# pqpeqr/RL-2048-with-Reinforce-and-Actor-Critic

Hardware: AMD Instinct MI355X
Metric: env steps/sec (whole node) + achieved HBM GB/s, batch=1M 4x4 boards (higher is better)
Workload: dtype u64

## Files before the change

rl-2048-with-reinforce-and-actor-critic_amd/csrc/g2048_dw2.hip:

```cpp
#include <hip/hip_runtime.h>

#include "g2048.h"

namespace {

typedef float floatx16 __attribute__((ext_vector_type(16)));
typedef __bf16 bf16x8 __attribute__((ext_vector_type(8)));

constexpr int kBK = 16;
constexpr int kAhead = 2;
constexpr int kStages = kAhead + 2;
constexpr int kThreads = 256;

__host__ __device__ inline int acc_row(int r, int h) { return (r & 3) + 8 * (r >> 2) + 4 * h; }

__device__ __forceinline__ void glds16(const float* src, float* lds_wave_base) {
#if defined(__HIP_DEVICE_COMPILE__)
    const uint32_t lds = __builtin_amdgcn_readfirstlane(
        (uint32_t)(uintptr_t)(__attribute__((address_space(3))) float*)lds_wave_base);
    uint32_t keep;
    asm volatile("s_mov_b32 %0, m0\n\ts_mov_b32 m0, %2\n\ts_nop 0\n\tglobal_load_lds_dwordx4 %1, off\n\ts_mov_b32 m0, %0"
                 : "=&s"(keep)
                 : "v"(src), "s"(lds)
                 : "memory");
#else
    (void)src;
    (void)lds_wave_base;
#endif
}

__host__ __device__ constexpr int dw2_threads(int nt2) { return nt2 >= 8 ? 512 : 256; }

template <int NT1, int NT2, int MODE>
struct Dw2 {
    static constexpr bool FAC = MODE != 0;
    static constexpr int H1 = 32 * NT1, H2 = 32 * NT2;
    static constexpr int RB = H1 > H2 ? H1 : H2;
    static constexpr bool WIDE = NT2 >= 8;
    static constexpr int CS = 1;
    static constexpr int kW = WIDE ? 8 : 4;
    static constexpr int WR = 2, WC = kW / 2;
    static constexpr int kThr = 64 * kW;
    static_assert(kThr == dw2_threads(NT2), "launch bounds");
    static constexpr int NT2h = NT2 / CS, H2h = H2 / CS;
    static constexpr int kRows = FAC ? H1 : H1 + H2h;
    static constexpr int kRecFloats = FAC ? 256 : 0;
    static constexpr int kStageFloats = kRows * kBK + kRecFloats;
    static constexpr int kRowGlds = kRows / 16;
    static constexpr int kGlds = kRowGlds + (FAC ? 1 : 0);
    static constexpr int kGldsPerWave = (kGlds + kW - 1) / kW;
    static constexpr int TR = NT1 >= WR ? NT1 / WR : 1;
    static constexpr int TC = NT2h >= WC ? NT2h / WC : 1;
};

struct Dw2Args {
    const float* a1t;
    const float* d2t;
    const float* w3;
    float* part;
    uint32_t ld, col0, ncols, kb;
};


__device__ __forceinline__ void split3(const float (&v)[8], bf16x8& p0, bf16x8& p1, bf16x8& p2) {
#pragma unroll
    for (int j = 0; j < 8; j++) {
        const __bf16 h = (__bf16)v[j];
        const float r = v[j] - (float)h;
        const __bf16 m = (__bf16)r;
        const float r2 = r - (float)m;
        p0[j] = h;
        p1[j] = m;
        p2[j] = (__bf16)r2;
    }
}

__device__ __forceinline__ void read_frag(const float* stage, int row, int h, float (&v)[8]) {
    const int f = (row >> 2) & 3;
    const float4 x = *reinterpret_cast<const float4*>(stage + row * kBK + (((2 * h) ^ f) << 2));
    const float4 y = *reinterpret_cast<const float4*>(stage + row * kBK + (((2 * h + 1) ^ f) << 2));
    v[0] = x.x; v[1] = x.y; v[2] = x.z; v[3] = x.w;
    v[4] = y.x; v[5] = y.y; v[6] = y.z; v[7] = y.w;
}

template <int NT1, int NT2, int MODE>
__global__ void __launch_bounds__(dw2_threads(NT2), 1) dw2_kernel(Dw2Args a) {
    using G = Dw2<NT1, NT2, MODE>;
    constexpr bool FAC = G::FAC;
    __shared__ float S[kStages * G::kStageFloats];
    const int t = threadIdx.x, lane = t & 63, w = t >> 6, h = lane >> 5, r = lane & 31;
    const int wr = w / G::WC, wc = w % G::WC;
    const uint32_t k_begin = a.col0 + blockIdx.x * a.kb;
    const uint32_t k_end = min(k_begin + a.kb, a.col0 + a.ncols);
    const int iters = k_end > k_begin ? (int)((k_end - k_begin) / kBK) : 0;
    const int c0 = (int)blockIdx.y * G::H2h;

    const int ws = __builtin_amdgcn_readfirstlane(w);
    const auto glds_index = [&](int i) {
        const int g = ws + G::kW * i;
        return g < G::kGlds ? g : G::kGlds - 1;
    };
    const float* src[G::kGldsPerWave];
#pragma unroll
    for (int i = 0; i < G::kGldsPerWave; i++) {
        const int g = glds_index(i);
        if (FAC && g == G::kRowGlds) {
            src[i] = a.d2t + (size_t)(k_begin / kBK) * 256 + 4 * lane;
        } else {
            const int row = 16 * g + (lane >> 2);
            const int chunk = (lane & 3) ^ ((lane >> 4) & 3);
            const float* base = row < G::H1 ? a.a1t + row * kBK : a.d2t + (row - G::H1 + c0) * kBK;
            src[i] = base + (size_t)(k_begin / kBK) * G::RB * kBK + 4 * chunk;
        }
    }
    const auto issue_to = [&](int slot, int stage_idx) {
        float* dst = S + slot * G::kStageFloats;
#pragma unroll
        for (int i = 0; i < G::kGldsPerWave; i++) {
            const int g = glds_index(i);
            const uint32_t stride = (FAC && g == G::kRowGlds) ? 256u : (uint32_t)(G::RB * kBK);
            glds16(src[i] + (size_t)stage_idx * stride, dst + 16 * g * kBK);
        }
    };

    floatx16 acc[G::TR][G::TC];
#pragma unroll
    for (int i = 0; i < G::TR; i++)
#pragma unroll
        for (int j = 0; j < G::TC; j++) acc[i][j] = floatx16{};
    const bool rows_mine = NT1 >= G::WR || wr == 0, cols_mine = G::NT2h >= G::WC || wc == 0;
    const int drow = G::H1 + (t < G::H2h ? t : G::H2h - 1);
    const int dunit = c0 + (t < G::H2h ? t : G::H2h - 1);
    float dsum = 0.0f;
    float4 w3d = make_float4(0.f, 0.f, 0.f, 0.f), w3c[G::TC];
    if constexpr (MODE == 2) {
        const float4* w3v = reinterpret_cast<const float4*>(a.w3);
        w3d = w3v[dunit];
#pragma unroll
        for (int j = 0; j < G::TC; j++) w3c[j] = w3v[c0 + 32 * ((G::NT2h >= G::WC ? wc : 0) * G::TC + j) + r];
    }
    const auto d2_of = [](const float4 g, const float4 w, bool m) {
        float dh = g.x * w.x;
        dh = fmaf(g.y, w.y, dh);
        dh = fmaf(g.z, w.z, dh);
        dh = fmaf(g.w, w.w, dh);
        return dh * (m ? 1.0f : 0.0f);
    };

    struct Planes {
        bf16x8 a0[G::TR], a1[G::TR], a2[G::TR], b0[G::TC], b1[G::TC], b2[G::TC];
    };
    typedef unsigned int u32x4 __attribute__((ext_vector_type(4)));
    const auto load = [&](const float* st, Planes& p) {
        if constexpr (MODE == 2) {
            const float* rec = st + G::kRows * kBK;
            const uint16_t* mw = reinterpret_cast<const uint16_t*>(rec);
            const float4* gv = reinterpret_cast<const float4*>(rec + 128);
            {
                const uint32_t m = mw[dunit];
#pragma unroll
                for (int e = 0; e < 16; e++) dsum += d2_of(gv[e], w3d, (m >> e) & 1u);
            }
            if (rows_mine && cols_mine) {
#pragma unroll
                for (int i = 0; i < G::TR; i++) {
                    float v[8];
                    read_frag(st, 32 * (wr * G::TR + i) + r, h, v);
                    split3(v, p.a0[i], p.a1[i], p.a2[i]);
                }
                float4 gk[8];
#pragma unroll
                for (int e = 0; e < 8; e++) gk[e] = gv[8 * h + e];
#pragma unroll
                for (int j = 0; j < G::TC; j++) {
                    const uint32_t m = (uint32_t)mw[c0 + 32 * (wc * G::TC + j) + r] >> (8 * h);
                    float v[8];
#pragma unroll
                    for (int e = 0; e < 8; e++) v[e] = d2_of(gk[e], w3c[j], (m >> e) & 1u);
                    split3(v, p.b0[j], p.b1[j], p.b2[j]);
                }
            }
            return;
        }
        if constexpr (MODE == 1) {
            const float* rec = st + G::kRows * kBK;
            const uint16_t* mw = reinterpret_cast<const uint16_t*>(rec);
            const float* gv = rec + 128;
            {
                const uint32_t m = mw[dunit];
#pragma unroll
                for (int c = 0; c < 4; c++) {
                    const float4 x = *reinterpret_cast<const float4*>(gv + 4 * c);
                    dsum += ((m >> (4 * c + 0)) & 1u) ? x.x : 0.0f;
                    dsum += ((m >> (4 * c + 1)) & 1u) ? x.y : 0.0f;
                    dsum += ((m >> (4 * c + 2)) & 1u) ? x.z : 0.0f;
                    dsum += ((m >> (4 * c + 3)) & 1u) ? x.w : 0.0f;
                }
            }
            if (rows_mine && cols_mine) {
                const float4 g0 = *reinterpret_cast<const float4*>(gv + 8 * h);
                const float4 g1 = *reinterpret_cast<const float4*>(gv + 8 * h + 4);
                const float gk[8] = {g0.x, g0.y, g0.z, g0.w, g1.x, g1.y, g1.z, g1.w};
#pragma unroll
                for (int i = 0; i < G::TR; i++) {
                    float v[8];
                    read_frag(st, 32 * (wr * G::TR + i) + r, h, v);
#pragma unroll
                    for (int e = 0; e < 8; e++) v[e] *= gk[e];
                    split3(v, p.a0[i], p.a1[i], p.a2[i]);
                }
#pragma unroll
                for (int j = 0; j < G::TC; j++) {
                    const uint32_t m = (uint32_t)mw[c0 + 32 * (wc * G::TC + j) + r] >> (8 * h);
                    u32x4 q;
#pragma unroll
                    for (int e = 0; e < 4; e++)
                        q[e] = (((m >> (2 * e)) & 1u) * 0x3F80u) | (((m >> (2 * e + 1)) & 1u) * 0x3F800000u);
                    p.b0[j] = __builtin_bit_cast(bf16x8, q);
                }
            }
            return;
        }
        const float* rowp = st + drow * kBK;
#pragma unroll
        for (int c = 0; c < 4; c++) {
            const float4 x = *reinterpret_cast<const float4*>(rowp + 4 * c);
            dsum += x.x;
            dsum += x.y;
            dsum += x.z;
            dsum += x.w;
        }
        if (rows_mine && cols_mine) {
#pragma unroll
            for (int i = 0; i < G::TR; i++) {
                float v[8];
                read_frag(st, 32 * (wr * G::TR + i) + r, h, v);
                split3(v, p.a0[i], p.a1[i], p.a2[i]);
            }
#pragma unroll
            for (int j = 0; j < G::TC; j++) {
                float v[8];
                read_frag(st, G::H1 + 32 * (wc * G::TC + j) + r, h, v);
                split3(v, p.b0[j], p.b1[j], p.b2[j]);
            }
        }
    };
    const auto mfma = [&](const Planes& p) {
        if (rows_mine && cols_mine) {
#pragma unroll
            for (int i = 0; i < G::TR; i++)
#pragma unroll
                for (int j = 0; j < G::TC; j++) {
                    floatx16 c = acc[i][j];
                    if constexpr (MODE == 1) {
                        c = __builtin_amdgcn_mfma_f32_32x32x16_bf16(p.a2[i], p.b0[j], c, 0, 0, 0);
                        c = __builtin_amdgcn_mfma_f32_32x32x16_bf16(p.a1[i], p.b0[j], c, 0, 0, 0);
                        c = __builtin_amdgcn_mfma_f32_32x32x16_bf16(p.a0[i], p.b0[j], c, 0, 0, 0);
                        acc[i][j] = c;
                        continue;
                    }
                    c = __builtin_amdgcn_mfma_f32_32x32x16_bf16(p.a2[i], p.b0[j], c, 0, 0, 0);
                    c = __builtin_amdgcn_mfma_f32_32x32x16_bf16(p.a1[i], p.b1[j], c, 0, 0, 0);
                    c = __builtin_amdgcn_mfma_f32_32x32x16_bf16(p.a0[i], p.b2[j], c, 0, 0, 0);
                    c = __builtin_amdgcn_mfma_f32_32x32x16_bf16(p.a1[i], p.b0[j], c, 0, 0, 0);
                    c = __builtin_amdgcn_mfma_f32_32x32x16_bf16(p.a0[i], p.b1[j], c, 0, 0, 0);
                    c = __builtin_amdgcn_mfma_f32_32x32x16_bf16(p.a0[i], p.b0[j], c, 0, 0, 0);
                    acc[i][j] = c;
                }
        }
    };
    const auto step = [&](int it, const Planes& cur, Planes& nxt) {
        const int q = it + 1 + kAhead;
        issue_to(q % kStages, q < iters ? q : iters - 1);
        asm volatile("s_waitcnt vmcnt(%0)" ::"n"(kAhead * G::kGldsPerWave) : "memory");
        __builtin_amdgcn_s_barrier();
        asm volatile("" ::: "memory");
        load(S + ((it + 1) % kStages) * G::kStageFloats, nxt);
        mfma(cur);
        constexpr int kMfma = (MODE == 1 ? 3 : 6) * G::TR * G::TC;
        __builtin_amdgcn_sched_group_barrier(0x100, 8, 0);
#pragma unroll
        for (int m = 0; m < kMfma; m++) {
            __builtin_amdgcn_sched_group_barrier(0x008, 1, 0);
            __builtin_amdgcn_sched_group_barrier(0x100, 1, 0);
            __builtin_amdgcn_sched_group_barrier(0x002, 4, 0);
        }
    };

    if constexpr (G::WIDE) {
        Planes pa;
        if (iters > 0) {
#pragma unroll
            for (int q = 0; q < kAhead; q++) issue_to(q, q < iters ? q : iters - 1);
            for (int it = 0; it < iters; it++) {
                const int q = it + kAhead;
                issue_to(q % kStages, q < iters ? q : iters - 1);
                asm volatile("s_waitcnt vmcnt(%0)" ::"n"(kAhead * G::kGldsPerWave) : "memory");
                __builtin_amdgcn_s_barrier();
                asm volatile("" ::: "memory");
                load(S + (it % kStages) * G::kStageFloats, pa);
                mfma(pa);
            }
            asm volatile("s_waitcnt vmcnt(0)" ::: "memory");
        }
    } else {
    Planes pa, pb;
    if (iters > 0) {
#pragma unroll
        for (int q = 0; q <= kAhead; q++) issue_to(q, q < iters ? q : iters - 1);
        asm volatile("s_waitcnt vmcnt(%0)" ::"n"(kAhead * G::kGldsPerWave) : "memory");
        __builtin_amdgcn_s_barrier();
        asm volatile("" ::: "memory");
        load(S, pa);
        int it = 0;
        for (; it + 2 < iters; it += 2) {
            step(it, pa, pb);
            step(it + 1, pb, pa);
        }
        if (it + 1 < iters) {
            step(it, pa, pb);
            mfma(pb);
        } else {
            mfma(pa);
        }
        asm volatile("s_waitcnt vmcnt(0)" ::: "memory");
    }
    }
    float* out = a.part + (size_t)blockIdx.x * (G::H1 + 1) * G::H2;
    if (rows_mine && cols_mine) {
#pragma unroll
        for (int j = 0; j < G::TC; j++) {
            const float ws = MODE == 1 ? a.w3[c0 + 32 * (wc * G::TC + j) + r] : 1.0f;
#pragma unroll
            for (int i = 0; i < G::TR; i++)
#pragma unroll
                for (int q = 0; q < 16; q++)
                    out[(size_t)(32 * (wr * G::TR + i) + acc_row(q, h)) * G::H2 + c0 + 32 * (wc * G::TC + j) + r] =
                        MODE == 1 ? acc[i][j][q] * ws : acc[i][j][q];
        }
    }
    if (t < G::H2h) out[(size_t)G::H1 * G::H2 + dunit] = MODE == 1 ? dsum * a.w3[dunit] : dsum;
}

template <int NT1, int MODE>
void launch_nt2(const Dw2Args& a, int nt2, int grid, hipStream_t s) {
    switch (nt2) {
        case 1: hipLaunchKernelGGL((dw2_kernel<NT1, 1, MODE>), dim3(grid, Dw2<NT1, 1, MODE>::CS), dim3(Dw2<NT1, 1, MODE>::kThr), 0, s, a); break;
        case 2: hipLaunchKernelGGL((dw2_kernel<NT1, 2, MODE>), dim3(grid, Dw2<NT1, 2, MODE>::CS), dim3(Dw2<NT1, 2, MODE>::kThr), 0, s, a); break;
        case 4: hipLaunchKernelGGL((dw2_kernel<NT1, 4, MODE>), dim3(grid, Dw2<NT1, 4, MODE>::CS), dim3(Dw2<NT1, 4, MODE>::kThr), 0, s, a); break;
        default: hipLaunchKernelGGL((dw2_kernel<NT1, 8, MODE>), dim3(grid, Dw2<NT1, 8, MODE>::CS), dim3(Dw2<NT1, 8, MODE>::kThr), 0, s, a); break;
    }
}

template <int NT1>
void launch_mode(const Dw2Args& a, int mode, int nt2, int grid, hipStream_t s) {
    if (mode == 1) launch_nt2<NT1, 1>(a, nt2, grid, s);
    else if (mode == 2) launch_nt2<NT1, 2>(a, nt2, grid, s);
    else launch_nt2<NT1, 0>(a, nt2, grid, s);
}

int tiles_of(int hsize) {
    const int t = (hsize + 31) / 32;
    return t <= 1 ? 1 : t <= 2 ? 2 : t <= 4 ? 4 : 8;
}

__global__ void __launch_bounds__(1024) fold_kernel(const float* __restrict__ part, uint32_t nparts, uint32_t slab,
                                                    double* __restrict__ acc) {
    __shared__ double ws[16][64];
    const uint32_t G = blockDim.x >> 6, g = threadIdx.x >> 6, e = threadIdx.x & 63u;
    const uint32_t i = blockIdx.x * 64u + e;
    const uint32_t ic = i < slab ? i : slab - 1u;
    double s = 0.0;
    uint32_t p = g;
    for (; p + 7u * G < nparts; p += 8u * G) {
        float v[8];
#pragma unroll
        for (int q = 0; q < 8; q++) v[q] = part[(size_t)(p + q * G) * slab + ic];
#pragma unroll
        for (int q = 0; q < 8; q++) s += (double)v[q];
    }
    for (; p < nparts; p += G) s += (double)part[(size_t)p * slab + ic];
    ws[g][e] = s;
    __syncthreads();
    if (g == 0 && i < slab) {
        double t = ws[0][e];
        for (uint32_t k = 1; k < G; k++) t += ws[k][e];
        acc[i] += t;
    }
}

}

namespace g2048_internal {
int set_error(int code, const char* msg);
}

static int dw2_launch(const float* a1t, const float* d2t, const float* w3, int mode, int h1, int h2, int64_t ld,
                      int64_t col0, int64_t ncols, int64_t cols_per_part, float* partials, int64_t nparts, void* stream) {
    using g2048_internal::set_error;
    if (h1 < 1 || h1 > 256 || h2 < 1 || h2 > 256) return set_error(G2048_EINVAL, "dw2: hidden sizes must be in 1..256");
    if (!a1t || !d2t || !partials || (mode && !w3)) return set_error(G2048_EINVAL, "dw2: NULL buffer");
    if (ld <= 0 || (ld & 15) || ld > ((int64_t)1 << 28)) return set_error(G2048_EINVAL, "dw2: ld must be a positive multiple of 16");
    if (col0 < 0 || (col0 & 15) || ncols < 0 || (ncols & 15) || col0 + ncols > ld)
        return set_error(G2048_EINVAL, "dw2: column range must be multiples of 16 inside ld");
    if (cols_per_part <= 0 || (cols_per_part & 15)) return set_error(G2048_EINVAL, "dw2: cols_per_part must be a positive multiple of 16");
    if (nparts != (ncols + cols_per_part - 1) / cols_per_part || nparts > 65535)
        return set_error(G2048_EINVAL, "dw2: nparts must be ceil(ncols / cols_per_part) (<= 65535)");
    if (nparts == 0) return G2048_OK;
    Dw2Args a{a1t, d2t, w3, partials, (uint32_t)ld, (uint32_t)col0, (uint32_t)ncols, (uint32_t)cols_per_part};
    const int nt1 = tiles_of(h1), nt2 = tiles_of(h2);
    hipStream_t s = (hipStream_t)stream;
    const int grid = (int)nparts;
    switch (nt1) {
        case 1: launch_mode<1>(a, mode, nt2, grid, s); break;
        case 2: launch_mode<2>(a, mode, nt2, grid, s); break;
        case 4: launch_mode<4>(a, mode, nt2, grid, s); break;
        default: launch_mode<8>(a, mode, nt2, grid, s); break;
    }
    const hipError_t e = hipGetLastError();
    if (e != hipSuccess) return set_error(G2048_EHIP, hipGetErrorString(e));
    return G2048_OK;
}

extern "C" int g2048_dw2(const float* a1t, const float* d2t, int h1, int h2, int64_t ld, int64_t col0, int64_t ncols,
                         int64_t cols_per_part, float* partials, int64_t nparts, void* stream) {
    return dw2_launch(a1t, d2t, nullptr, 0, h1, h2, ld, col0, ncols, cols_per_part, partials, nparts, stream);
}

extern "C" int g2048_dw2_factored(const float* a1t, const float* records, const float* w3, int h1, int h2, int64_t ld,
                                  int64_t col0, int64_t ncols, int64_t cols_per_part, float* partials, int64_t nparts,
                                  void* stream) {
    return dw2_launch(a1t, records, w3, 1, h1, h2, ld, col0, ncols, cols_per_part, partials, nparts, stream);
}

extern "C" int g2048_dw2_actor(const float* a1t, const float* records, const float* w3, int h1, int h2, int64_t ld,
                               int64_t col0, int64_t ncols, int64_t cols_per_part, float* partials, int64_t nparts,
                               void* stream) {
    return dw2_launch(a1t, records, w3, 2, h1, h2, ld, col0, ncols, cols_per_part, partials, nparts, stream);
}

extern "C" int g2048_fold_partials(const float* partials, int64_t nparts, int64_t slab, double* acc, void* stream) {
    using g2048_internal::set_error;
    if (!partials || !acc) return set_error(G2048_EINVAL, "fold_partials: NULL buffer");
    if (nparts < 0 || slab < 0 || nparts > ((int64_t)1 << 24) || slab > ((int64_t)1 << 28))
        return set_error(G2048_EINVAL, "fold_partials: nparts / slab out of range");
    if (nparts == 0 || slab == 0) return G2048_OK;
    const int64_t blocks = (slab + 63) / 64;
    int G = 1;
    while (G < 16 && blocks * G < 4096 && nparts >= 16 * G) G *= 2;
    hipLaunchKernelGGL(fold_kernel, dim3((unsigned)blocks), dim3(64 * G), 0, (hipStream_t)stream, partials,
                       (uint32_t)nparts, (uint32_t)slab, acc);
    const hipError_t e = hipGetLastError();
    if (e != hipSuccess) return set_error(G2048_EHIP, hipGetErrorString(e));
    return G2048_OK;
}
```

Measured before the change: 34.59 billion.

## Cooperatively pre-split LDS tiles into bf16 planes once per stage in dw2 kernel

```diff
diff --git a/rl-2048-with-reinforce-and-actor-critic_amd/csrc/g2048_dw2.hip b/rl-2048-with-reinforce-and-actor-critic_amd/csrc/g2048_dw2.hip
--- a/rl-2048-with-reinforce-and-actor-critic_amd/csrc/g2048_dw2.hip
+++ b/rl-2048-with-reinforce-and-actor-critic_amd/csrc/g2048_dw2.hip
@@ -1,15 +1,19 @@
 #include <hip/hip_runtime.h>
 
 #include "g2048.h"
+#include "g2048_dw2_layout.h"
 
 namespace {
+
+namespace LY = dw2_layout;
 
 typedef float floatx16 __attribute__((ext_vector_type(16)));
 typedef __bf16 bf16x8 __attribute__((ext_vector_type(8)));
 
-constexpr int kBK = 16;
+constexpr int kBK = LY::kBK;
 constexpr int kAhead = 2;
 constexpr int kStages = kAhead + 2;
+static_assert(kStages == LY::kStages, "g2048_dw2_layout.h");
 constexpr int kThreads = 256;
 
 __host__ __device__ inline int acc_row(int r, int h) { return (r & 3) + 8 * (r >> 2) + 4 * h; }
@@ -29,7 +33,7 @@
 #endif
 }
 
-__host__ __device__ constexpr int dw2_threads(int nt2) { return nt2 >= 8 ? 512 : 256; }
+__host__ __device__ constexpr int dw2_threads(int nt2) { return LY::threads(nt2); }
 
 template <int NT1, int NT2, int MODE>
 struct Dw2 {
@@ -37,6 +41,7 @@
     static constexpr int H1 = 32 * NT1, H2 = 32 * NT2;
     static constexpr int RB = H1 > H2 ? H1 : H2;
     static constexpr bool WIDE = NT2 >= 8;
+    static constexpr bool COOP = LY::coop(NT2, MODE);
     static constexpr int CS = 1;
     static constexpr int kW = WIDE ? 8 : 4;
     static constexpr int WR = 2, WC = kW / 2;
@@ -46,6 +51,11 @@
     static constexpr int kRows = FAC ? H1 : H1 + H2h;
     static constexpr int kRecFloats = FAC ? 256 : 0;
     static constexpr int kStageFloats = kRows * kBK + kRecFloats;
+    static constexpr int kSideFloats = LY::side_floats(NT1, NT2, MODE);
+    static constexpr int kLdsFloats = LY::lds_floats(NT1, NT2, MODE);
+    static_assert(kRows == LY::rows(NT1, NT2, MODE) && kStageFloats == LY::stage_floats(NT1, NT2, MODE),
+                  "g2048_dw2_layout.h");
+    static_assert(kLdsFloats * 4 <= LY::kLdsBytes, "LDS");
     static constexpr int kRowGlds = kRows / 16;
     static constexpr int kGlds = kRowGlds + (FAC ? 1 : 0);
     static constexpr int kGldsPerWave = (kGlds + kW - 1) / kW;
@@ -76,9 +86,8 @@
 }
 
 __device__ __forceinline__ void read_frag(const float* stage, int row, int h, float (&v)[8]) {
-    const int f = (row >> 2) & 3;
-    const float4 x = *reinterpret_cast<const float4*>(stage + row * kBK + (((2 * h) ^ f) << 2));
-    const float4 y = *reinterpret_cast<const float4*>(stage + row * kBK + (((2 * h + 1) ^ f) << 2));
+    const float4 x = *reinterpret_cast<const float4*>(stage + LY::chunk_off(row, 2 * h));
+    const float4 y = *reinterpret_cast<const float4*>(stage + LY::chunk_off(row, 2 * h + 1));
     v[0] = x.x; v[1] = x.y; v[2] = x.z; v[3] = x.w;
     v[4] = y.x; v[5] = y.y; v[6] = y.z; v[7] = y.w;
 }
@@ -87,7 +96,7 @@
 __global__ void __launch_bounds__(dw2_threads(NT2), 1) dw2_kernel(Dw2Args a) {
     using G = Dw2<NT1, NT2, MODE>;
     constexpr bool FAC = G::FAC;
-    __shared__ float S[kStages * G::kStageFloats];
+    __shared__ float S[G::kLdsFloats];
     const int t = threadIdx.x, lane = t & 63, w = t >> 6, h = lane >> 5, r = lane & 31;
     const int wr = w / G::WC, wc = w % G::WC;
     const uint32_t k_begin = a.col0 + blockIdx.x * a.kb;
@@ -129,8 +138,11 @@
 #pragma unroll
         for (int j = 0; j < G::TC; j++) acc[i][j] = floatx16{};
     const bool rows_mine = NT1 >= G::WR || wr == 0, cols_mine = G::NT2h >= G::WC || wc == 0;
-    const int drow = G::H1 + (t < G::H2h ? t : G::H2h - 1);
-    const int dunit = c0 + (t < G::H2h ? t : G::H2h - 1);
+    constexpr bool kRowDb2 = G::COOP && MODE == 0;
+    const bool db2_mine = kRowDb2 ? (t >= G::H1 && t < G::kRows) : t < G::H2h;
+    const int du = kRowDb2 ? t - G::H1 : t;
+    const int drow = G::H1 + (db2_mine ? du : G::H2h - 1);
+    const int dunit = c0 + (db2_mine ? du : G::H2h - 1);
     float dsum = 0.0f;
     float4 w3d = make_float4(0.f, 0.f, 0.f, 0.f), w3c[G::TC];
     if constexpr (MODE == 2) {
@@ -151,7 +163,61 @@
         bf16x8 a0[G::TR], a1[G::TR], a2[G::TR], b0[G::TC], b1[G::TC], b2[G::TC];
     };
     typedef unsigned int u32x4 __attribute__((ext_vector_type(4)));
-    const auto load = [&](const float* st, Planes& p) {
+    const auto planes_of = [&](const float* st, const float* sd, int row, const float* gk, bf16x8& p0, bf16x8& p1,
+                               bf16x8& p2) {
+        if constexpr (G::COOP) {
+            p0 = *reinterpret_cast<const bf16x8*>(st + LY::plane01_off(row, h, 0));
+            p1 = *reinterpret_cast<const bf16x8*>(st + LY::plane01_off(row, h, 1));
+            p2 = *reinterpret_cast<const bf16x8*>(sd + LY::plane2_off(row, h));
+        } else {
+            float v[8];
+            read_frag(st, row, h, v);
+            if (gk) {
+#pragma unroll
+                for (int e = 0; e < 8; e++) v[e] *= gk[e];
+            }
+            split3(v, p0, p1, p2);
+        }
+    };
+    const auto convert = [&](float* st, float* sd, bool live) {
+        if constexpr (G::COOP) {
+            constexpr bool kAll = LY::conv_items(NT1, NT2, MODE, G::kThr - 1) != 0;
+            if (!kAll && LY::conv_items(NT1, NT2, MODE, t) == 0) return;
+            if constexpr (MODE == 0) {
+                const float* rowp = st + t * kBK;
+                float ds = dsum;
+#pragma unroll
+                for (int c = 0; c < 4; c++) {
+                    const float4 x = *reinterpret_cast<const float4*>(rowp + 4 * c);
+                    ds += x.x;
+                    ds += x.y;
+                    ds += x.z;
+                    ds += x.w;
+                }
+                dsum = live ? ds : dsum;
+            }
+#pragma unroll
+            for (int k = 0; k < (MODE == 0 ? 2 : 1); k++) {
+                const int row = LY::conv_row(NT1, MODE, t, k), hh = LY::conv_half(NT1, MODE, t, k);
+                float v[8];
+                read_frag(st, row, hh, v);
+                if constexpr (MODE == 1) {
+                    const float* gv = st + G::kRows * kBK + 128 + 8 * hh;
+                    const float4 g0 = *reinterpret_cast<const float4*>(gv);
+                    const float4 g1 = *reinterpret_cast<const float4*>(gv + 4);
+                    const float gk[8] = {g0.x, g0.y, g0.z, g0.w, g1.x, g1.y, g1.z, g1.w};
+#pragma unroll
+                    for (int e = 0; e < 8; e++) v[e] *= gk[e];
+                }
+                bf16x8 p0, p1, p2;
+                split3(v, p0, p1, p2);
+                *reinterpret_cast<bf16x8*>(st + LY::plane01_off(row, hh, 0)) = p0;
+                *reinterpret_cast<bf16x8*>(st + LY::plane01_off(row, hh, 1)) = p1;
+                *reinterpret_cast<bf16x8*>(sd + LY::plane2_off(row, hh)) = p2;
+            }
+        }
+    };
+    const auto load = [&](const float* st, const float* sd, Planes& p) {
         if constexpr (MODE == 2) {
             const float* rec = st + G::kRows * kBK;
             const uint16_t* mw = reinterpret_cast<const uint16_t*>(rec);
@@ -163,11 +229,8 @@
             }
             if (rows_mine && cols_mine) {
 #pragma unroll
-                for (int i = 0; i < G::TR; i++) {
-                    float v[8];
-                    read_frag(st, 32 * (wr * G::TR + i) + r, h, v);
-                    split3(v, p.a0[i], p.a1[i], p.a2[i]);
-                }
+                for (int i = 0; i < G::TR; i++)
+                    planes_of(st, sd, 32 * (wr * G::TR + i) + r, nullptr, p.a0[i], p.a1[i], p.a2[i]);
                 float4 gk[8];
 #pragma unroll
                 for (int e = 0; e < 8; e++) gk[e] = gv[8 * h + e];
@@ -186,7 +249,7 @@
             const float* rec = st + G::kRows * kBK;
             const uint16_t* mw = reinterpret_cast<const uint16_t*>(rec);
             const float* gv = rec + 128;
-            {
+            const auto db2 = [&] {
                 const uint32_t m = mw[dunit];
 #pragma unroll
                 for (int c = 0; c < 4; c++) {
@@ -196,19 +259,22 @@
                     dsum += ((m >> (4 * c + 2)) & 1u) ? x.z : 0.0f;
                     dsum += ((m >> (4 * c + 3)) & 1u) ? x.w : 0.0f;
                 }
-            }
-            if (rows_mine && cols_mine) {
-                const float4 g0 = *reinterpret_cast<const float4*>(gv + 8 * h);
-                const float4 g1 = *reinterpret_cast<const float4*>(gv + 8 * h + 4);
-                const float gk[8] = {g0.x, g0.y, g0.z, g0.w, g1.x, g1.y, g1.z, g1.w};
-#pragma unroll
-                for (int i = 0; i < G::TR; i++) {
-                    float v[8];
-                    read_frag(st, 32 * (wr * G::TR + i) + r, h, v);
-#pragma unroll
-                    for (int e = 0; e < 8; e++) v[e] *= gk[e];
-                    split3(v, p.a0[i], p.a1[i], p.a2[i]);
-                }
+            };
+            const auto a_frags = [&] {
+                if constexpr (G::COOP) {
+#pragma unroll
+                    for (int i = 0; i < G::TR; i++)
+                        planes_of(st, sd, 32 * (wr * G::TR + i) + r, nullptr, p.a0[i], p.a1[i], p.a2[i]);
+                } else {
+                    const float4 g0 = *reinterpret_cast<const float4*>(gv + 8 * h);
+                    const float4 g1 = *reinterpret_cast<const float4*>(gv + 8 * h + 4);
+                    const float gk[8] = {g0.x, g0.y, g0.z, g0.w, g1.x, g1.y, g1.z, g1.w};
+#pragma unroll
+                    for (int i = 0; i < G::TR; i++)
+                        planes_of(st, sd, 32 * (wr * G::TR + i) + r, gk, p.a0[i], p.a1[i], p.a2[i]);
+                }
+            };
+            const auto b_frags = [&] {
 #pragma unroll
                 for (int j = 0; j < G::TC; j++) {
                     const uint32_t m = (uint32_t)mw[c0 + 32 * (wc * G::TC + j) + r] >> (8 * h);
@@ -218,30 +284,46 @@
                         q[e] = (((m >> (2 * e)) & 1u) * 0x3F80u) | (((m >> (2 * e + 1)) & 1u) * 0x3F800000u);
                     p.b0[j] = __builtin_bit_cast(bf16x8, q);
                 }
+            };
+            if constexpr (G::COOP) {
+                if (rows_mine && cols_mine) {
+                    b_frags();
+                    a_frags();
+                }
+                db2();
+            } else {
+                db2();
+                if (rows_mine && cols_mine) {
+                    a_frags();
+                    b_frags();
+                }
             }
             return;
         }
-        const float* rowp = st + drow * kBK;
-#pragma unroll
-        for (int c = 0; c < 4; c++) {
-            const float4 x = *reinterpret_cast<const float4*>(rowp + 4 * c);
-            dsum += x.x;
-            dsum += x.y;
-            dsum += x.z;
-            dsum += x.w;
+        if constexpr (!G::COOP) {
+            const float* rowp = st + drow * kBK;
+#pragma unroll
+            for (int c = 0; c < 4; c++) {
+                const float4 x = *reinterpret_cast<const float4*>(rowp + 4 * c);
+                dsum += x.x;
+                dsum += x.y;
+                dsum += x.z;
+                dsum += x.w;
+            }
         }
         if (rows_mine && cols_mine) {
-#pragma unroll
-            for (int i = 0; i < G::TR; i++) {
-                float v[8];
-                read_frag(st, 32 * (wr * G::TR + i) + r, h, v);
-                split3(v, p.a0[i], p.a1[i], p.a2[i]);
-            }
-#pragma unroll
-            for (int j = 0; j < G::TC; j++) {
-                float v[8];
-                read_frag(st, G::H1 + 32 * (wc * G::TC + j) + r, h, v);
-                split3(v, p.b0[j], p.b1[j], p.b2[j]);
+            if constexpr (G::COOP) {
+#pragma unroll
+                for (int j = 0; j < G::TC; j++)
+                    planes_of(st, sd, G::H1 + 32 * (wc * G::TC + j) + r, nullptr, p.b0[j], p.b1[j], p.b2[j]);
+            }
+#pragma unroll
+            for (int i = 0; i < G::TR; i++)
+                planes_of(st, sd, 32 * (wr * G::TR + i) + r, nullptr, p.a0[i], p.a1[i], p.a2[i]);
+            if constexpr (!G::COOP) {
+#pragma unroll
+                for (int j = 0; j < G::TC; j++)
+                    planes_of(st, sd, G::H1 + 32 * (wc * G::TC + j) + r, nullptr, p.b0[j], p.b1[j], p.b2[j]);
             }
         }
     };
@@ -275,7 +357,7 @@
         asm volatile("s_waitcnt vmcnt(%0)" ::"n"(kAhead * G::kGldsPerWave) : "memory");
         __builtin_amdgcn_s_barrier();
         asm volatile("" ::: "memory");
-        load(S + ((it + 1) % kStages) * G::kStageFloats, nxt);
+        load(S + ((it + 1) % kStages) * G::kStageFloats, nullptr, nxt);
         mfma(cur);
         constexpr int kMfma = (MODE == 1 ? 3 : 6) * G::TR * G::TC;
         __builtin_amdgcn_sched_group_barrier(0x100, 8, 0);
@@ -287,7 +369,34 @@
         }
     };
 
-    if constexpr (G::WIDE) {
+    if constexpr (G::COOP) {
+        Planes pa;
+        float* const sides = S + kStages * G::kStageFloats;
+        if (iters > 0) {
+#pragma unroll
+            for (int q = 0; q <= kAhead; q++) issue_to(q, q < iters ? q : iters - 1);
+            asm volatile("s_waitcnt vmcnt(%0)" ::"n"(kAhead * G::kGldsPerWave) : "memory");
+            __builtin_amdgcn_s_barrier();
+            asm volatile("" ::: "memory");
+            convert(S, sides, true);
+            for (int it = 0; it < iters; it++) {
+                asm volatile("s_waitcnt vmcnt(%0) lgkmcnt(0)" ::"n"((kAhead - 1) * G::kGldsPerWave) : "memory");
+                __builtin_amdgcn_s_barrier();
+                asm volatile("" ::: "memory");
+                const int q = it + 1 + kAhead;
+                issue_to(q % kStages, q < iters ? q : iters - 1);
+                float* const cst = S + ((it + 1) % kStages) * G::kStageFloats;
+                float* const csd = sides + ((it + 1) & 1) * G::kSideFloats;
+                if (ws < G::kW / 2) convert(cst, csd, it + 1 < iters);
+                __builtin_amdgcn_sched_barrier(0);
+                load(S + (it % kStages) * G::kStageFloats, sides + (it & 1) * G::kSideFloats, pa);
+                mfma(pa);
+                __builtin_amdgcn_sched_barrier(0);
+                if (ws >= G::kW / 2) convert(cst, csd, it + 1 < iters);
+            }
+            asm volatile("s_waitcnt vmcnt(0) lgkmcnt(0)" ::: "memory");
+        }
+    } else if constexpr (G::WIDE) {
         Planes pa;
         if (iters > 0) {
 #pragma unroll
@@ -298,7 +407,7 @@
                 asm volatile("s_waitcnt vmcnt(%0)" ::"n"(kAhead * G::kGldsPerWave) : "memory");
                 __builtin_amdgcn_s_barrier();
                 asm volatile("" ::: "memory");
-                load(S + (it % kStages) * G::kStageFloats, pa);
+                load(S + (it % kStages) * G::kStageFloats, nullptr, pa);
                 mfma(pa);
             }
             asm volatile("s_waitcnt vmcnt(0)" ::: "memory");
@@ -311,7 +420,7 @@
         asm volatile("s_waitcnt vmcnt(%0)" ::"n"(kAhead * G::kGldsPerWave) : "memory");
         __builtin_amdgcn_s_barrier();
         asm volatile("" ::: "memory");
-        load(S, pa);
+        load(S, nullptr, pa);
         int it = 0;
         for (; it + 2 < iters; it += 2) {
             step(it, pa, pb);
@@ -339,7 +448,7 @@
                         MODE == 1 ? acc[i][j][q] * ws : acc[i][j][q];
         }
     }
-    if (t < G::H2h) out[(size_t)G::H1 * G::H2 + dunit] = MODE == 1 ? dsum * a.w3[dunit] : dsum;
+    if (db2_mine) out[(size_t)G::H1 * G::H2 + dunit] = MODE == 1 ? dsum * a.w3[dunit] : dsum;
 }
 
 template <int NT1, int MODE>
diff --git a/rl-2048-with-reinforce-and-actor-critic_amd/csrc/g2048_dw2_layout.h b/rl-2048-with-reinforce-and-actor-critic_amd/csrc/g2048_dw2_layout.h
--- /dev/null
+++ b/rl-2048-with-reinforce-and-actor-critic_amd/csrc/g2048_dw2_layout.h
@@ -0,0 +1,41 @@
+#pragma once
+
+#if defined(__HIPCC__) || defined(__CUDACC__)
+#define DW2_HD __host__ __device__
+#else
+#define DW2_HD
+#endif
+
+namespace dw2_layout {
+
+constexpr int kBK = 16;
+constexpr int kStages = 4;
+constexpr int kSides = 2;
+constexpr int kLdsBytes = 160 * 1024;
+
+DW2_HD constexpr int threads(int nt2) { return nt2 >= 8 ? 512 : 256; }
+DW2_HD constexpr bool wide(int nt2) { return nt2 >= 8; }
+#ifndef G2048_DW2_COOP_COLUMNS
+#define G2048_DW2_COOP_COLUMNS 0
+#endif
+DW2_HD constexpr bool coop(int nt2, int mode) {
+    return wide(nt2) && (mode == 1 || (mode == 0 && G2048_DW2_COOP_COLUMNS != 0));
+}
+DW2_HD constexpr int rows(int nt1, int nt2, int mode) { return mode ? 32 * nt1 : 32 * nt1 + 32 * nt2; }
+DW2_HD constexpr int stage_floats(int nt1, int nt2, int mode) { return rows(nt1, nt2, mode) * kBK + (mode ? 256 : 0); }
+DW2_HD constexpr int side_floats(int nt1, int nt2, int mode) { return coop(nt2, mode) ? rows(nt1, nt2, mode) * 8 : 0; }
+DW2_HD constexpr int lds_floats(int nt1, int nt2, int mode) {
+    return kStages * stage_floats(nt1, nt2, mode) + kSides * side_floats(nt1, nt2, mode);
+}
+
+DW2_HD constexpr int chunk_off(int row, int chunk) { return row * kBK + ((chunk ^ ((row >> 2) & 3)) << 2); }
+DW2_HD constexpr int plane01_off(int row, int half, int plane) { return chunk_off(row, 2 * half + plane); }
+DW2_HD constexpr int plane2_off(int row, int half) { return row * 8 + ((half ^ ((row >> 3) & 1)) << 2); }
+
+DW2_HD constexpr int conv_items(int nt1, int nt2, int mode, int t) {
+    return !coop(nt2, mode) ? 0 : mode ? (t < 64 * nt1 ? 1 : 0) : (t < rows(nt1, nt2, mode) ? 2 : 0);
+}
+DW2_HD constexpr int conv_row(int nt1, int mode, int t, int ) { return mode ? t % (32 * nt1) : t; }
+DW2_HD constexpr int conv_half(int nt1, int mode, int t, int k) { return mode ? t / (32 * nt1) : k; }
+
+}
```

New measurement: 34.10 billion. -1.4%, worse.
